# Fro116/RecommenderSystem

Measured on AMD Instinct MI355X. Metric: interactions/sec, higher is better.
Workload: dtype bf16

## Files before the change

recommendersystem_amd/csrc/elementwise.hip:

```cpp
#include "kernels.hpp"

namespace rsys {

thread_local DetScratch g_det;

__global__ void reduce_parts_kernel(const float* __restrict__ part, int nparts, long long stride, int n, float* dst) {
  const int c = blockIdx.x * blockDim.x + threadIdx.x;
  if (c >= n) return;
  float acc = 0.f;
  for (int b = 0; b < nparts; ++b) acc += part[(long long)b * stride + c];
  dst[c] += acc;
}
__global__ void reduce_parts_stage_kernel(const float* __restrict__ part, int nparts, long long stride, int n, float* out) {
  const int c = blockIdx.x * blockDim.x + threadIdx.x, chunk = blockIdx.y;
  if (c >= n) return;
  const int b0 = chunk * 32, b1 = min(nparts, b0 + 32);
  float acc = 0.f;
  for (int b = b0; b < b1; ++b) acc += part[(long long)b * stride + c];
  out[(long long)chunk * n + c] = acc;
}
int launch_reduce_parts(const float* part, int nparts, long long stride, int n, float* dst, hipStream_t s) {
  if (nparts <= 0 || n <= 0) return RSYS_OK;
  if (nparts > 64 && g_det.tmp != nullptr) {
    const int chunks = (nparts + 31) / 32;
// ... 429 lines not shown
template int launch_dropout<float>(const float*, float*, long long, float, unsigned long long, unsigned int, int, hipStream_t);

struct SelectBatch { const float* w[4]; int* idx[4]; float* stats[4]; int* npos[4]; };
__global__ __launch_bounds__(1024) void select_positions_kernel(SelectBatch sb, int N, int topk) {
  const float* __restrict__ w = sb.w[blockIdx.x];
  int* idx = sb.idx[blockIdx.x]; float* stats = sb.stats[blockIdx.x]; int* npos_out = sb.npos[blockIdx.x];
  __shared__ int wave_tot[16];
  __shared__ float red[16];
  const int t = threadIdx.x, l = t & 63, wv = t >> 6;
  const int per = (N + 1023) / 1024;
  const int i0 = t * per, i1 = min(N, i0 + per);
  int cnt = 0; float wall = 0.f;
  for (int i = i0; i < i1; ++i) { float x = w[i]; cnt += x > 0.f; wall += x; }
  int inc = cnt;
#pragma unroll
  for (int o = 1; o < 64; o <<= 1) { int v = __shfl_up(inc, o, 64); if (l >= o) inc += v; }
  if (l == 63) wave_tot[wv] = inc;
  __syncthreads();
  int base = 0, npos = 0;
  for (int k = 0; k < 16; ++k) { int v = wave_tot[k]; if (k < wv) base += v; npos += v; }
  int rank = base + inc - cnt;
  float wsel = 0.f;
  for (int i = i0; i < i1; ++i) {
    float x = w[i];
    int slot = x > 0.f ? rank : npos + (i - rank);
    if (slot < topk) { idx[slot] = i; wsel += x; }
    rank += x > 0.f;
  }
  wsel = block_sum(wsel, red);
  wall = block_sum(wall, red);
  if (t == 0) { stats[0] = wsel; stats[1] = wall; if (npos_out) *npos_out = min(npos, topk); }
}
constexpr int SEL_CHUNKS = 32;
__global__ __launch_bounds__(256) void select_count_kernel(SelectBatch sb, int N, int* __restrict__ counts, float* __restrict__ wsums) {
  __shared__ float red[16];
  const int task = blockIdx.x / SEL_CHUNKS, ch = blockIdx.x % SEL_CHUNKS;
  const float* __restrict__ w = sb.w[task];
  const int per = (N + SEL_CHUNKS - 1) / SEL_CHUNKS, i0 = ch * per, i1 = min(N, i0 + per);
  float cnt = 0.f, wall = 0.f;
  for (int i = i0 + threadIdx.x; i < i1; i += 256) { const float x = w[i]; cnt += x > 0.f ? 1.f : 0.f; wall += x; }
  cnt = block_sum(cnt, red);
  wall = block_sum(wall, red);
  if (threadIdx.x == 0) { counts[blockIdx.x] = (int)cnt; wsums[blockIdx.x] = wall; }
}
__global__ __launch_bounds__(256) void select_place_kernel(SelectBatch sb, int N, int topk, const int* __restrict__ counts, const float* __restrict__ wsums,
                                                           float* __restrict__ wsel_part) {
  __shared__ int wave_tot[4];
  __shared__ float red[16];
  const int task = blockIdx.x / SEL_CHUNKS, ch = blockIdx.x % SEL_CHUNKS;
  const float* __restrict__ w = sb.w[task];
  int* idx = sb.idx[task];
  const int t = threadIdx.x, l = t & 63, wv = t >> 6;
  int before = 0, npos = 0;
  for (int k = 0; k < SEL_CHUNKS; ++k) { const int v = counts[task * SEL_CHUNKS + k]; if (k < ch) before += v; npos += v; }
  const int per = (N + SEL_CHUNKS - 1) / SEL_CHUNKS, i0 = ch * per, i1 = min(N, i0 + per);
  float wsel = 0.f;
  int rank0 = before;
  for (int j0 = i0; j0 < i1; j0 += 256) {
    const int i = j0 + t;
    const float x = i < i1 ? w[i] : 0.f;
    const int pos = x > 0.f ? 1 : 0;
    int inc = pos;
#pragma unroll
    for (int o = 1; o < 64; o <<= 1) { const int v = __shfl_up(inc, o, 64); if (l >= o) inc += v; }
    __syncthreads();
    if (l == 63) wave_tot[wv] = inc;
    __syncthreads();
    int base = 0, tot = 0;
#pragma unroll
    for (int k = 0; k < 4; ++k) { const int v = wave_tot[k]; if (k < wv) base += v; tot += v; }
    const int rank = rank0 + base + inc - pos;
    if (i < i1) {
      const int slot = pos ? rank : npos + (i - rank);
      if (slot < topk) { idx[slot] = i; wsel += x; }
    }
    rank0 += tot;
  }
  wsel = block_sum(wsel, red);
  if (t == 0) wsel_part[blockIdx.x] = wsel;
}
__global__ void select_finish_kernel(SelectBatch sb, int ntask, int topk, const int* __restrict__ counts, const float* __restrict__ wsums,
                                     const float* __restrict__ wsel_part) {
  const int task = threadIdx.x;
  if (task >= ntask) return;
  int npos = 0; float wall = 0.f, wsel = 0.f;
  for (int k = 0; k < SEL_CHUNKS; ++k) { npos += counts[task * SEL_CHUNKS + k]; wall += wsums[task * SEL_CHUNKS + k]; wsel += wsel_part[task * SEL_CHUNKS + k]; }
  sb.stats[task][0] = wsel; sb.stats[task][1] = wall;
  if (sb.npos[task]) *sb.npos[task] = min(npos, topk);
}
int launch_select_positions_chunked(int ntask, const float* const* w, int N, int topk, int* const* idx, float* const* stats, int* const* npos_out,
                                    void* scratch, hipStream_t s) {
  ARG_CHECK(topk <= N && ntask >= 1 && ntask <= 4 && scratch != nullptr, "select_positions: topk > N or more than 4 tasks");
  SelectBatch sb{};
  for (int i = 0; i < ntask; ++i) { sb.w[i] = w[i]; sb.idx[i] = idx[i]; sb.stats[i] = stats[i]; sb.npos[i] = npos_out[i]; }
  int* counts = (int*)scratch; float* wsums = (float*)scratch + 4 * SEL_CHUNKS; float* wsel = (float*)scratch + 8 * SEL_CHUNKS;
  hipLaunchKernelGGL(select_count_kernel, dim3(ntask * SEL_CHUNKS), dim3(256), 0, s, sb, N, counts, wsums);
  hipLaunchKernelGGL(select_place_kernel, dim3(ntask * SEL_CHUNKS), dim3(256), 0, s, sb, N, topk, counts, wsums, wsel);
  hipLaunchKernelGGL(select_finish_kernel, dim3(1), dim3(64), 0, s, sb, ntask, topk, counts, wsums, wsel);
  HIP_CHECK(hipGetLastError());
  return RSYS_OK;
}

int launch_select_positions(const float* w, int N, int topk, int* idx, float* stats, int* npos_out, hipStream_t s) {
  const float* ws[1] = {w}; int* is[1] = {idx}; float* st[1] = {stats}; int* np[1] = {npos_out};
  return launch_select_positions_batch(1, ws, N, topk, is, st, np, s);
}
int launch_select_positions_batch(int ntask, const float* const* w, int N, int topk, int* const* idx, float* const* stats,
                                  int* const* npos_out, hipStream_t s) {
  ARG_CHECK(topk <= N && ntask >= 1 && ntask <= 4, "select_positions: topk > N or more than 4 tasks");
  SelectBatch sb{};
  for (int i = 0; i < ntask; ++i) { sb.w[i] = w[i]; sb.idx[i] = idx[i]; sb.stats[i] = stats[i]; sb.npos[i] = npos_out[i]; }
  hipLaunchKernelGGL(select_positions_kernel, dim3(ntask), dim3(1024), 0, s, sb, N, topk);
  HIP_CHECK(hipGetLastError());
  return RSYS_OK;
}

template <typename T>
__global__ void gather_rows_kernel(const T* __restrict__ src, long long ld, const int* __restrict__ idx, int parity, T* dst, int n, int D) {
  const int row = (blockIdx.x * blockDim.x + threadIdx.x) >> 6, l = threadIdx.x & 63;
  if (row >= n) return;
  constexpr int E = 16 / sizeof(T);
  const uint4* s4 = (const uint4*)(src + (2LL * idx[row] + parity) * ld);
  uint4* d4 = (uint4*)(dst + (long long)row * D);
  for (int c = l; c < D / E; c += 64) d4[c] = s4[c];
}
template <typename T>
int launch_gather_rows(const T* src, long long ld, const int* idx, int parity, T* dst, int n, int D, hipStream_t s) {
  ARG_CHECK((D * sizeof(T)) % 16 == 0 && (ld * sizeof(T)) % 16 == 0, "gather_rows: rows must be 16-byte multiples");
  hipLaunchKernelGGL((gather_rows_kernel<T>), dim3(div_up(n, 4)), dim3(256), 0, s, src, ld, idx, parity, dst, n, D);
  HIP_CHECK(hipGetLastError());
  return RSYS_OK;
}
template int launch_gather_rows<bf16>(const bf16*, long long, const int*, int, bf16*, int, int, hipStream_t);
template int launch_gather_rows<float>(const float*, long long, const int*, int, float*, int, int, hipStream_t);

__global__ void scatter_rows_add_kernel(const float* __restrict__ src, const int* __restrict__ idx, int parity, float* dst, long long ld, int n, int D,
                                        const int* __restrict__ npos) {
  const int row = (blockIdx.x * blockDim.x + threadIdx.x) >> 6, l = threadIdx.x & 63;
  if (row >= n || (npos != nullptr && row >= *npos)) return;
  const float4* s4 = (const float4*)(src + (long long)row * D);
  float4* d4 = (float4*)(dst + (2LL * idx[row] + parity) * ld);
  for (int c = l; c < (D >> 2); c += 64) {
    float4 a = d4[c], b = s4[c];
    a.x += b.x; a.y += b.y; a.z += b.z; a.w += b.w;
    d4[c] = a;
  }
}
int launch_scatter_rows_add(const float* src, const int* idx, int parity, float* dst, long long ld, int n, int D, hipStream_t s, const int* npos) {
  hipLaunchKernelGGL(scatter_rows_add_kernel, dim3(div_up(n, 4)), dim3(256), 0, s, src, idx, parity, dst, ld, n, D, npos);
  HIP_CHECK(hipGetLastError());
  return RSYS_OK;
}

template <typename T>
__global__ __launch_bounds__(256) void ce_kernel(T* logits, long long ldl, int V, const int* __restrict__ idx,
                                                 const float* __restrict__ label, const float* __restrict__ weight,
                                                 const int* __restrict__ position, const float* __restrict__ stats,
                                                 const int* __restrict__ npos, float task_w, float* loss_out, float* part) {
  __shared__ float red[16];
  constexpr int E = 16 / sizeof(T);
  const int row = blockIdx.x, t = threadIdx.x;
  if (npos != nullptr && row >= ((*npos + 127) & ~127)) return;
  T* lr = logits + (long long)row * ldl;
  const int i = idx[row];
  const float w = weight[i], lab = label[i];
  const int nchunks = (int)(ldl / E);
  const float lw = lab * w;
  if (lw == 0.f) {
    for (int c = t; c < nchunks; c += 256) ((uint4*)lr)[c] = make_uint4(0, 0, 0, 0);
    return;
  }
  float m = -3.0e38f, ssum = 0.f;
  for (int c = t; c < nchunks; c += 256) {
    uint4 raw = ((const uint4*)lr)[c];
    const T* e = (const T*)&raw;
#pragma unroll
    for (int k = 0; k < E; ++k) {
      if (c * E + k < V) {
        float x = to_f32(e[k]);
        if (x > m) { ssum = ssum * __expf(m - x) + 1.f; m = x; }
        else ssum += __expf(x - m);
      }
    }
  }
  const float gm = block_max(m, red);
  ssum = block_sum(ssum * __expf(m - gm), red);
  const float lse = gm + logf(ssum);
  const int tgt = position[i];
  const float xt = to_f32(lr[tgt]);
  __syncthreads();
  if (t == 0) {
    if (part != nullptr) part[row] = (lse - xt) * lw;
    else atomicAdd(loss_out, (lse - xt) * lw);
  }
  const float coef = task_w * lw / fmaxf(stats[0], 1e-8f);
  for (int c = t; c < nchunks; c += 256) {
    uint4 raw = ((const uint4*)lr)[c];
    T* e = (T*)&raw;
#pragma unroll
    for (int k = 0; k < E; ++k) {
      int col = c * E + k;
      float x = to_f32(e[k]);
      float gl = col < V ? coef * (__expf(x - lse) - (col == tgt ? 1.f : 0.f)) : 0.f;
      e[k] = from_f32<T>(gl);
    }
    ((uint4*)lr)[c] = raw;
  }
}
template <typename T>
int launch_ce_fwd_bwd(T* logits, long long ldl, int n, int V, const int* idx, const float* label, const float* weight,
                      const int* position, const float* stats, const int* npos, float task_w, float* loss_out, hipStream_t s) {
  ARG_CHECK((ldl * sizeof(T)) % 16 == 0 && ldl >= V, "ce: ldl");
  if (n <= 0) return RSYS_OK;
  float* part = det_part(n);
  if (part != nullptr) HIP_CHECK(hipMemsetAsync(part, 0, (size_t)n * 4, s));
  hipLaunchKernelGGL((ce_kernel<T>), dim3(n), dim3(256), 0, s, logits, ldl, V, idx, label, weight, position, stats, npos, task_w, loss_out, part);
  HIP_CHECK(hipGetLastError());
  if (part != nullptr) return launch_reduce_parts(part, n, 1, 1, loss_out, s);
  return RSYS_OK;
}
template int launch_ce_fwd_bwd<bf16>(bf16*, long long, int, int, const int*, const float*, const float*, const int*, const float*, const int*, float, float*, hipStream_t);
template int launch_ce_fwd_bwd<float>(float*, long long, int, int, const int*, const float*, const float*, const int*, const float*, const int*, float, float*, hipStream_t);

template <typename T>
__global__ __launch_bounds__(256) void rating_tail_kernel(T* z, const T* __restrict__ hact, int n, int D,
                                                          const float* __restrict__ w2, const float* __restrict__ b2,
                                                          const int* __restrict__ idx, const float* __restrict__ label,
                                                          const float* __restrict__ weight, const float* __restrict__ stats,
                                                          float rating_mean, float task_w, int evaluate, float* loss_out,
                                                          float* dw2, float* db2, float* db0, float* part, const int* __restrict__ npos) {
  extern __shared__ __attribute__((aligned(16))) float sds[];
  const int l = threadIdx.x & 63, w = threadIdx.x >> 6;
  const int nacc = part != nullptr ? 4 * 2 * D + 16 : 2 * D;
  for (int c = threadIdx.x; c < nacc; c += 256) sds[c] = 0.f;
  __syncthreads();
  float* const mine = part != nullptr ? sds + w * 2 * D : sds;
  float l0 = 0.f, l1 = 0.f, l2 = 0.f, gb2 = 0.f;
  const float inv_ws = 1.f / fmaxf(stats[0], 1e-8f);
  if (npos != nullptr) n = min(n, (*npos + 127) & ~127);
  for (int row = blockIdx.x * 4 + w; row < n; row += gridDim.x * 4) {
    const int i = idx[row];
    const float wt = weight[i], tgt = label[i] - rating_mean;
    const T* hr = hact + (long long)row * D;
    T* zr = z + (long long)row * D;
    float acc = 0.f;
    for (int c = l; c < D; c += 64) acc += to_f32(hr[c]) * w2[c];
    acc = wave_sum(acc);
    const float pred = acc + b2[0];
    const float e1 = pred - tgt;
    l0 += e1 * e1 * wt; l1 += tgt * tgt * wt; l2 += (-pred - tgt) * (-pred - tgt) * wt;
    const float dpred = evaluate ? 0.f : task_w * 2.f * e1 * wt * inv_ws;
    gb2 += dpred;
    for (int c = l; c < D; c += 64) {
      float zz = to_f32(zr[c]);
      float gp = 0.5f * (1.f + erff(zz * 0.70710678118654752f)) + zz * __expf(-0.5f * zz * zz) * 0.3989422804014327f;
      float dz = dpred * w2[c] * gp;
      zr[c] = from_f32<T>(dz);
      if (dpred != 0.f) {
        if (part != nullptr) { mine[c] += dpred * to_f32(hr[c]); mine[D + c] += dz; }
        else { atomicAdd(&sds[c], dpred * to_f32(hr[c])); atomicAdd(&sds[D + c], dz); }
      }
    }
  }
  if (part != nullptr) {
    float* sc = sds + 4 * 2 * D;
    if (l == 0) { sc[w * 4 + 0] = gb2; sc[w * 4 + 1] = l0; sc[w * 4 + 2] = l1; sc[w * 4 + 3] = l2; }
    __syncthreads();
    float* pr = part + (long long)blockIdx.x * (2 * D + 4);
    for (int c = threadIdx.x; c < 2 * D; c += 256) pr[c] = ((sds[c] + sds[2 * D + c]) + sds[4 * D + c]) + sds[6 * D + c];
    if (threadIdx.x < 4) pr[2 * D + threadIdx.x] = ((sc[threadIdx.x] + sc[4 + threadIdx.x]) + sc[8 + threadIdx.x]) + sc[12 + threadIdx.x];
    return;
  }
  __syncthreads();
  if (!evaluate) {
    for (int c = threadIdx.x; c < D; c += 256) {
      if (sds[c] != 0.f) atomicAdd(&dw2[c], sds[c]);
      if (sds[D + c] != 0.f) atomicAdd(&db0[c], sds[D + c]);
    }
    if (l == 0 && gb2 != 0.f) atomicAdd(db2, gb2);
  }
  if (l == 0) {
    if (l0 != 0.f) atomicAdd(&loss_out[0], l0);
    if (l1 != 0.f) atomicAdd(&loss_out[1], l1);
    if (l2 != 0.f) atomicAdd(&loss_out[2], l2);
  }
}
template <typename T>
int launch_rating_tail(T* z, const T* hact, int n, int D, const float* w2, const float* b2, const int* idx,
                       const float* label, const float* weight, const float* stats, float rating_mean, float task_w,
                       int evaluate, float* loss_out, float* dw2, float* db2, float* db0, hipStream_t s, const int* npos) {
  if (n <= 0) return RSYS_OK;
  int grid = std::min(div_up(n, 4), 512);
  const long long prow = 2LL * D + 4;
  float* part = det_part(grid * prow);
  hipLaunchKernelGGL((rating_tail_kernel<T>), dim3(grid), dim3(256), (part ? 8 * D + 16 : 2 * D) * sizeof(float), s, z, hact, n, D, w2, b2, idx,
                     label, weight, stats, rating_mean, task_w, evaluate, loss_out, dw2, db2, db0, part, npos);
  HIP_CHECK(hipGetLastError());
  if (part != nullptr) {
    int rc = RSYS_OK;
    if (!evaluate) {
      rc = launch_reduce_parts(part, grid, prow, D, dw2, s);
      if (rc == RSYS_OK) rc = launch_reduce_parts(part + D, grid, prow, D, db0, s);
      if (rc == RSYS_OK) rc = launch_reduce_parts(part + 2 * D, grid, prow, 1, db2, s);
    }
    return rc == RSYS_OK ? launch_reduce_parts(part + 2 * D + 1, grid, prow, 3, loss_out, s) : rc;
  }
  return RSYS_OK;
}
template int launch_rating_tail<bf16>(bf16*, const bf16*, int, int, const float*, const float*, const int*, const float*, const float*, const float*, float, float, int, float*, float*, float*, float*, hipStream_t, const int*);
template int launch_rating_tail<float>(float*, const float*, int, int, const float*, const float*, const int*, const float*, const float*, const float*, float, float, int, float*, float*, float*, float*, hipStream_t, const int*);

template <typename T>
__global__ void widen_kernel(const T* __restrict__ src, float* __restrict__ dst, long long n) {
  for (long long i = (long long)blockIdx.x * blockDim.x + threadIdx.x; i < n; i += (long long)gridDim.x * blockDim.x) dst[i] = to_f32(src[i]);
}
template <typename T>
int launch_widen(const T* src, float* dst, long long n, hipStream_t s) {
  const int blocks = (int)std::min<long long>((n + 255) / 256, 8192);
  hipLaunchKernelGGL((widen_kernel<T>), dim3(blocks), dim3(256), 0, s, src, dst, n);
  HIP_CHECK(hipGetLastError());
  return RSYS_OK;
}
template int launch_widen<bf16>(const bf16*, float*, long long, hipStream_t);
template int launch_widen<float>(const float*, float*, long long, hipStream_t);
template <typename T>
__global__ void rowdot_kernel(const T* __restrict__ h, const float* __restrict__ w, const float* __restrict__ b, float* out, int n, int D) {
  const int row = (blockIdx.x * blockDim.x + threadIdx.x) >> 6, l = threadIdx.x & 63;
  if (row >= n) return;
  const T* hr = h + (long long)row * D;
  float acc = 0.f;
  for (int c = l; c < D; c += 64) acc += to_f32(hr[c]) * w[c];
  acc = wave_sum(acc);
  if (l == 0) out[row] = acc + b[0];
}
template <typename T>
int launch_rowdot(const T* h, const float* w, const float* b, float* out, int n, int D, hipStream_t s) {
  hipLaunchKernelGGL((rowdot_kernel<T>), dim3(div_up(n, 4)), dim3(256), 0, s, h, w, b, out, n, D);
  HIP_CHECK(hipGetLastError());
  return RSYS_OK;
}
template int launch_rowdot<bf16>(const bf16*, const float*, const float*, float*, int, int, hipStream_t);
template int launch_rowdot<float>(const float*, const float*, const float*, float*, int, int, hipStream_t);

template <typename TS>
__global__ void colsum_kernel(const TS* __restrict__ src, long long ld, long long rows, int cols, float* dst, int rows_per_block, float* part) {
  const int c = blockIdx.x * blockDim.x + threadIdx.x;
  if (c >= cols) return;
  const long long r0 = (long long)blockIdx.y * rows_per_block, r1 = min(rows, r0 + rows_per_block);
  float acc = 0.f;
  for (long long r = r0; r < r1; ++r) acc += to_f32(src[r * ld + c]);
  if (part != nullptr) part[(long long)blockIdx.y * cols + c] = acc;
  else if (acc != 0.f) atomicAdd(&dst[c], acc);
}
template <typename TS>
static int colsum_any(const TS* src, long long ld, long long rows, int cols, float* dst, hipStream_t s) {
  int rpb = (int)std::max<long long>(64, (rows + 511) / 512);
  dim3 grid(div_up(cols, 256), div_up(rows, rpb));
  float* part = det_part((long long)grid.y * cols);
  hipLaunchKernelGGL((colsum_kernel<TS>), grid, dim3(256), 0, s, src, ld, rows, cols, dst, rpb, part);
  HIP_CHECK(hipGetLastError());
  if (part != nullptr) return launch_reduce_parts(part, (int)grid.y, cols, cols, dst, s);
  return RSYS_OK;
}
int launch_colsum_add(const float* src, long long ld, long long rows, int cols, float* dst, hipStream_t s) {
  return colsum_any<float>(src, ld, rows, cols, dst, s);
}

__global__ __launch_bounds__(1024) void cast_colsum_kernel(const float* __restrict__ src, bf16* __restrict__ dst, long long rows, int D,
                                                           float* colsum, int rows_per_block, float* part) {
  __shared__ float red[2048];
  const int cg = D >> 2;
  const int c = (threadIdx.x % cg) * 4, lane_r = threadIdx.x / cg, nr = 1024 / cg;
  const long long r0 = (long long)blockIdx.x * rows_per_block, r1 = min(rows, r0 + rows_per_block);
  float4 acc = make_float4(0, 0, 0, 0);
  long long r = r0 + lane_r;
  for (; r + 3 * nr < r1; r += 4 * nr) {
    float4 v[4];
#pragma unroll
    for (int u = 0; u < 4; ++u) v[u] = *(const float4*)(src + (r + u * nr) * D + c);
#pragma unroll
    for (int u = 0; u < 4; ++u) {
      bf16x4 o; o[0] = (bf16)v[u].x; o[1] = (bf16)v[u].y; o[2] = (bf16)v[u].z; o[3] = (bf16)v[u].w;
      *(bf16x4*)(dst + (r + u * nr) * D + c) = o;
      acc.x += v[u].x; acc.y += v[u].y; acc.z += v[u].z; acc.w += v[u].w;
    }
  }
  for (; r < r1; r += nr) {
    const float4 v = *(const float4*)(src + r * D + c);
    bf16x4 o; o[0] = (bf16)v.x; o[1] = (bf16)v.y; o[2] = (bf16)v.z; o[3] = (bf16)v.w;
    *(bf16x4*)(dst + r * D + c) = o;
    acc.x += v.x; acc.y += v.y; acc.z += v.z; acc.w += v.w;
  }
  if (lane_r < 2) *(float4*)&red[lane_r * D + c] = acc;
  __syncthreads();
  for (int base = 2; base < nr; base += 2) {
    if (lane_r >= base && lane_r < base + 2) {
      float4 o = *(float4*)&red[(lane_r - base) * D + c];
      o.x += acc.x; o.y += acc.y; o.z += acc.z; o.w += acc.w;
      *(float4*)&red[(lane_r - base) * D + c] = o;
    }
    __syncthreads();
  }
  for (int cc = threadIdx.x; cc < D; cc += 1024) {
    const float v = red[cc] + (nr > 1 ? red[D + cc] : 0.f);
    if (part != nullptr) part[(long long)blockIdx.x * D + cc] = v;
    else if (v != 0.f) atomicAdd(&colsum[cc], v);
  }
}
int launch_cast_colsum(const float* src, bf16* dst, long long rows, int D, float* colsum, hipStream_t s) {
  ARG_CHECK(D % 4 == 0 && D <= 1024 && 1024 % (D >> 2) == 0, "cast_colsum: D/4 must divide 1024, D <= 1024");
  const int rpb = (int)std::max<long long>(32, (rows + 511) / 512);
  const int grid = div_up(rows, rpb);
  float* part = det_part((long long)grid * D);
  hipLaunchKernelGGL(cast_colsum_kernel, dim3(grid), dim3(1024), 0, s, src, dst, rows, D, colsum, rpb, part);
  HIP_CHECK(hipGetLastError());
  if (part != nullptr) return launch_reduce_parts(part, grid, D, D, colsum, s);
  return RSYS_OK;
}

__global__ __launch_bounds__(256) void cast_transpose_colsum_kernel(const float* __restrict__ src, bf16* __restrict__ dstT, long long rows, int D,
                                                                    long long ldt, float* colsum, int rows_per_block, float* part) {
  __shared__ unsigned short tile[64][72];
  __shared__ float red[16][64];
  const int t = threadIdx.x;
  const int lr = t >> 4, c4 = (t & 15) * 4;
  const int oc = t >> 2, or8 = (t & 3) * 16;
  const long long r0 = (long long)blockIdx.x * rows_per_block;
  const long long rend = min((rows + 63) & ~63LL, r0 + rows_per_block);
  for (int ct = 0; ct < D / 64; ++ct) {
    float4 acc = make_float4(0, 0, 0, 0);
    for (long long rb = r0; rb < rend; rb += 64) {
      float4 v[4];
#pragma unroll
      for (int i = 0; i < 4; ++i) {
        const long long r = rb + 4 * lr + i;
        v[i] = r < rows ? *(const float4*)(src + r * D + ct * 64 + c4) : make_float4(0, 0, 0, 0);
        acc.x += v[i].x; acc.y += v[i].y; acc.z += v[i].z; acc.w += v[i].w;
      }
      {
        bf16x4 o;
        o[0] = (bf16)v[0].x; o[1] = (bf16)v[1].x; o[2] = (bf16)v[2].x; o[3] = (bf16)v[3].x; *(bf16x4*)&tile[c4 + 0][4 * lr] = o;
        o[0] = (bf16)v[0].y; o[1] = (bf16)v[1].y; o[2] = (bf16)v[2].y; o[3] = (bf16)v[3].y; *(bf16x4*)&tile[c4 + 1][4 * lr] = o;
        o[0] = (bf16)v[0].z; o[1] = (bf16)v[1].z; o[2] = (bf16)v[2].z; o[3] = (bf16)v[3].z; *(bf16x4*)&tile[c4 + 2][4 * lr] = o;
        o[0] = (bf16)v[0].w; o[1] = (bf16)v[1].w; o[2] = (bf16)v[2].w; o[3] = (bf16)v[3].w; *(bf16x4*)&tile[c4 + 3][4 * lr] = o;
      }
      __syncthreads();
      {
        const uint4 q0 = *(const uint4*)&tile[oc][or8], q1 = *(const uint4*)&tile[oc][or8 + 8];
        uint4* d = (uint4*)(dstT + (long long)(ct * 64 + oc) * ldt + rb + or8);
        d[0] = q0; d[1] = q1;
      }
      __syncthreads();
    }
    *(float4*)&red[lr][c4] = acc;
    __syncthreads();
    if (t < 64) {
      float v = 0.f;
#pragma unroll
      for (int k = 0; k < 16; ++k) v += red[k][t];
      if (part != nullptr) part[(long long)blockIdx.x * D + ct * 64 + t] = v;
      else if (v != 0.f) atomicAdd(&colsum[ct * 64 + t], v);
    }
    __syncthreads();
  }
}
int launch_cast_transpose_colsum(const float* src, bf16* dstT, long long rows, int D, long long ldt, float* colsum, hipStream_t s) {
  ARG_CHECK(D % 64 == 0 && ldt % 8 == 0 && ldt >= ((rows + 63) & ~63LL), "cast_transpose_colsum: D % 64, ldt % 8, ldt >= rows rounded up to 64");
  const long long chunks = (rows + 63) / 64;
  const int cpb = (int)std::max<long long>(1, (chunks + 2047) / 2048);
  const int grid = (int)((chunks + cpb - 1) / cpb);
  float* part = det_part((long long)grid * D);
  hipLaunchKernelGGL(cast_transpose_colsum_kernel, dim3(grid), dim3(256), 0, s, src, dstT, rows, D, ldt, colsum, cpb * 64, part);
  HIP_CHECK(hipGetLastError());
  if (part != nullptr) return launch_reduce_parts(part, grid, D, D, colsum, s);
  return RSYS_OK;
}

__global__ void embedding_scatter_kernel(const float* __restrict__ gx0, BatchDev b, int V, int D, float* gE) {
  const int n = (blockIdx.x * blockDim.x + threadIdx.x) >> 6, l = threadIdx.x & 63;
  if (n >= b.N) return;
  int id = b.m_matchedid[n];
  id = id == -1 ? V : id;
  const float* src = gx0 + (long long)(2 * n) * D;
  float* dst = gE + (long long)id * D;
  for (int c = l; c < D; c += 64) atomicAdd(&dst[c], src[c]);
}
int launch_embedding_scatter_add(const float* gx0, const BatchDev& b, int V, int D, float* gE, hipStream_t s) {
  hipLaunchKernelGGL(embedding_scatter_kernel, dim3(div_up(b.N, 4)), dim3(256), 0, s, gx0, b, V, D, gE);
  HIP_CHECK(hipGetLastError());
  return RSYS_OK;
}

__global__ __launch_bounds__(256) void action_small_bwd_kernel(const float* __restrict__ gf, BatchDev b, SmallParams sp,
                                                               float* g_cos, float* g_sin, float* g_status, float* g_gender,
                                                               float* g_source) {
  __shared__ float acc[4 + 16 * 4 + 16 * 4 + 16 * 16];
  const int NG = (sp.n_gender + 1) * 4, NS = (sp.n_source + 1) * 4, NST = (sp.n_status + 1) * 16;
  float* a_g = acc + 4; float* a_s = a_g + 64; float* a_st = a_s + 64;
  for (int c = threadIdx.x; c < 4 + 64 + 64 + 256; c += 256) acc[c] = 0.f;
  __syncthreads();
  for (int i = blockIdx.x * blockDim.x + threadIdx.x; i < b.N; i += gridDim.x * blockDim.x) {
    const float* g = gf + (long long)i * 32;
    float p0, p1; double ts;
    periodic_args(b.time[i], sp.min_ts, p0, p1, ts);
    atomicAdd(&acc[0], -sinf(p0 + sp.per_cos[0]) * g[1]);
    atomicAdd(&acc[1], -sinf(p1 + sp.per_cos[1]) * g[2]);
    atomicAdd(&acc[2], cosf(p0 + sp.per_sin[0]) * g[3]);
    atomicAdd(&acc[3], cosf(p1 + sp.per_sin[1]) * g[4]);
    int gi = b.gender[i]; gi = gi == -1 ? sp.n_gender : gi;
    int si = b.source[i]; si = si == -1 ? sp.n_source : si;
    int st = b.m_status[i]; st = st == -1 ? sp.n_status : st;
#pragma unroll
    for (int k = 0; k < 4; ++k) atomicAdd(&a_g[gi * 4 + k], g[5 + k]);
#pragma unroll
    for (int k = 0; k < 4; ++k) atomicAdd(&a_s[si * 4 + k], g[9 + k]);
#pragma unroll
    for (int k = 0; k < 16; ++k) atomicAdd(&a_st[st * 16 + k], g[15 + k]);
  }
// ... 58 lines not shown
```

Baseline: 1.631 million.

## Register-resident CE kernel, vectorized rating tail, and float4 column-sum kernel

The cross-entropy kernel now keeps the whole logit row in registers across larger blocks. It computes max and sum-exp in separate passes rather than with an online rescale, and writes gradients without re-reading global memory. The rating tail kernel vectorizes its loads and keeps w2 and the per-lane accumulators in registers, replacing shared-memory atomics with a per-wave serialized reduction on a smaller grid. A new float4 colsum kernel uses a shared-memory row reduction for the nondeterministic path; the deterministic paths keep the older kernels, and the changes add register pressure and more template variants.

```diff
diff --git a/recommendersystem_amd/csrc/elementwise.hip b/recommendersystem_amd/csrc/elementwise.hip
--- a/recommendersystem_amd/csrc/elementwise.hip
+++ b/recommendersystem_amd/csrc/elementwise.hip
@@ -605,36 +605,92 @@
   return RSYS_OK;
 }
 
-template <typename T>
-__global__ __launch_bounds__(256) void ce_kernel(T* logits, long long ldl, int V, const int* __restrict__ idx,
-                                                 const float* __restrict__ label, const float* __restrict__ weight,
-                                                 const int* __restrict__ position, const float* __restrict__ stats,
-                                                 const int* __restrict__ npos, float task_w, float* loss_out, float* part) {
+constexpr float CE_NEG = -3.0e38f;
+
+__device__ __forceinline__ bool ce_row_skipped(int row, const int* __restrict__ npos) {
+  return npos != nullptr && row >= ((*npos + 127) & ~127);
+}
+__device__ __forceinline__ void ce_clear_row(void* lr, int nchunks) {
+  for (int c = threadIdx.x; c < nchunks; c += blockDim.x) ((uint4*)lr)[c] = make_uint4(0, 0, 0, 0);
+}
+__device__ __forceinline__ unsigned& ce_word(uint4& q, int j) { return j == 0 ? q.x : j == 1 ? q.y : j == 2 ? q.z : q.w; }
+template <typename T>
+__device__ __forceinline__ float ce_get(uint4& q, int k) {
+  if constexpr (is_bf16<T>::value) return __uint_as_float(k & 1 ? ce_word(q, k >> 1) & 0xffff0000u : ce_word(q, k >> 1) << 16);
+  else return __uint_as_float(ce_word(q, k));
+}
+template <typename T>
+__device__ __forceinline__ void ce_set_neg(uint4& q, int k) {
+  if constexpr (is_bf16<T>::value) ce_word(q, k >> 1) = k & 1 ? (ce_word(q, k >> 1) & 0xffffu) | 0xff620000u : (ce_word(q, k >> 1) & 0xffff0000u) | 0xff62u;
+  else ce_word(q, k) = __float_as_uint(CE_NEG);
+}
+template <typename T>
+__device__ __forceinline__ void ce_grad_chunk(uint4& raw, int cbase, int V, int tgt, float lse, float coef) {
+  constexpr int E = 16 / sizeof(T);
+  float g[E];
+  if ((unsigned)(tgt - cbase) >= (unsigned)E && cbase + E <= V) {
+#pragma unroll
+    for (int k = 0; k < E; ++k) g[k] = coef * (__expf(ce_get<T>(raw, k) - lse) - 0.f);
+  } else {
+#pragma unroll
+    for (int k = 0; k < E; ++k) {
+      const int col = cbase + k;
+      const float gl = coef * (__expf(ce_get<T>(raw, k) - lse) - (col == tgt ? 1.f : 0.f));
+      g[k] = col < V ? gl : 0.f;
+    }
+  }
+#pragma unroll
+  for (int j = 0; j < 4; ++j) {
+    if constexpr (is_bf16<T>::value) { bf16x2 pk; pk[0] = (bf16)g[2 * j]; pk[1] = (bf16)g[2 * j + 1]; ce_word(raw, j) = __builtin_bit_cast(unsigned, pk); }
+    else ce_word(raw, j) = __float_as_uint(g[j]);
+  }
+}
+
+__device__ __forceinline__ void ce_tie(float& a, uint4& q) {
+  asm volatile("" : "+v"(a), "+v"(q.x), "+v"(q.y), "+v"(q.z), "+v"(q.w));
+}
+
+template <typename T, int NT, int NC>
+__global__ __launch_bounds__(NT) void ce_kernel(T* logits, long long ldl, int V, const int* __restrict__ idx,
+                                                const float* __restrict__ label, const float* __restrict__ weight,
+                                                const int* __restrict__ position, const float* __restrict__ stats,
+                                                const int* __restrict__ npos, float task_w, float* loss_out, float* part) {
   __shared__ float red[16];
   constexpr int E = 16 / sizeof(T);
   const int row = blockIdx.x, t = threadIdx.x;
-  if (npos != nullptr && row >= ((*npos + 127) & ~127)) return;
+  if (ce_row_skipped(row, npos)) return;
   T* lr = logits + (long long)row * ldl;
   const int i = idx[row];
-  const float w = weight[i], lab = label[i];
-  const int nchunks = (int)(ldl / E);
-  const float lw = lab * w;
-  if (lw == 0.f) {
-    for (int c = t; c < nchunks; c += 256) ((uint4*)lr)[c] = make_uint4(0, 0, 0, 0);
-    return;
-  }
-  float m = -3.0e38f, ssum = 0.f;
-  for (int c = t; c < nchunks; c += 256) {
-    uint4 raw = ((const uint4*)lr)[c];
-    const T* e = (const T*)&raw;
-#pragma unroll
-    for (int k = 0; k < E; ++k) {
-      if (c * E + k < V) {
-        float x = to_f32(e[k]);
-        if (x > m) { ssum = ssum * __expf(m - x) + 1.f; m = x; }
-        else ssum += __expf(x - m);
-      }
-    }
+  const int nchunks = (int)(ldl / E), vchunks = (V + E - 1) / E;
+  const float lw = label[i] * weight[i];
+  if (lw == 0.f) { ce_clear_row(lr, nchunks); return; }
+  uint4 r[NC];
+#pragma unroll
+  for (int u = 0; u < NC; ++u) {
+    r[u] = ((const uint4*)lr)[min(t + u * NT, vchunks - 1)];
+  }
+  float m = CE_NEG;
+#pragma unroll
+  for (int u = 0; u < NC; ++u) {
+    const int cbase = (t + u * NT) * E;
+    ce_tie(m, r[u]);
+    if (cbase + E > V) {
+#pragma unroll
+      for (int k = 0; k < E; ++k) if (cbase + k >= V) ce_set_neg<T>(r[u], k);
+    }
+    float m0 = ce_get<T>(r[u], 0), m1 = ce_get<T>(r[u], 1);
+#pragma unroll
+    for (int k = 2; k < E; k += 2) { m0 = fmaxf(m0, ce_get<T>(r[u], k)); m1 = fmaxf(m1, ce_get<T>(r[u], k + 1)); }
+    m = fmaxf(m, fmaxf(m0, m1));
+  }
+  float ssum = 0.f;
+#pragma unroll
+  for (int u = 0; u < NC; ++u) {
+    ce_tie(ssum, r[u]);
+    float s0 = __expf(ce_get<T>(r[u], 0) - m), s1 = __expf(ce_get<T>(r[u], 1) - m);
+#pragma unroll
+    for (int k = 2; k < E; k += 2) { s0 += __expf(ce_get<T>(r[u], k) - m); s1 += __expf(ce_get<T>(r[u], k + 1) - m); }
+    ssum += s0 + s1;
   }
   const float gm = block_max(m, red);
   ssum = block_sum(ssum * __expf(m - gm), red);
@@ -646,20 +702,78 @@
     if (part != nullptr) part[row] = (lse - xt) * lw;
     else atomicAdd(loss_out, (lse - xt) * lw);
   }
+  float coef = task_w * lw / fmaxf(stats[0], 1e-8f);
+#pragma unroll
+  for (int u = 0; u < NC; ++u) {
+    const int c = t + u * NT;
+    ce_tie(coef, r[u]);
+    if (c < vchunks) {
+      ce_grad_chunk<T>(r[u], c * E, V, tgt, lse, coef);
+      ((uint4*)lr)[c] = r[u];
+    }
+  }
+  for (int c = vchunks + t; c < nchunks; c += NT) ((uint4*)lr)[c] = make_uint4(0, 0, 0, 0);
+}
+
+constexpr int CE2_NT = 256, CE2_U = 4;
+template <typename T>
+__global__ __launch_bounds__(CE2_NT) void ce_two_pass_kernel(T* logits, long long ldl, int V, const int* __restrict__ idx,
+                                                             const float* __restrict__ label, const float* __restrict__ weight,
+                                                             const int* __restrict__ position, const float* __restrict__ stats,
+                                                             const int* __restrict__ npos, float task_w, float* loss_out, float* part) {
+  __shared__ float red[16];
+  constexpr int E = 16 / sizeof(T);
+  const int row = blockIdx.x, t = threadIdx.x;
+  if (ce_row_skipped(row, npos)) return;
+  T* lr = logits + (long long)row * ldl;
+  const int i = idx[row];
+  const int nchunks = (int)(ldl / E);
+  const float lw = label[i] * weight[i];
+  if (lw == 0.f) { ce_clear_row(lr, nchunks); return; }
+  float m = -3.0e38f, ssum = 0.f;
+  for (int c0 = t; c0 < nchunks; c0 += CE2_U * CE2_NT) {
+    uint4 raw[CE2_U];
+#pragma unroll
+    for (int u = 0; u < CE2_U; ++u) raw[u] = ((const uint4*)lr)[min(c0 + u * CE2_NT, nchunks - 1)];
+#pragma unroll
+    for (int u = 0; u < CE2_U; ++u) {
+      const int c = c0 + u * CE2_NT;
+#pragma unroll
+      for (int k = 0; k < E; ++k) {
+        if (c < nchunks && c * E + k < V) {
+          float x = ce_get<T>(raw[u], k);
+          if (x > m) { ssum = ssum * __expf(m - x) + 1.f; m = x; }
+          else ssum += __expf(x - m);
+        }
+      }
+    }
+  }
+  const float gm = block_max(m, red);
+  ssum = block_sum(ssum * __expf(m - gm), red);
+  const float lse = gm + logf(ssum);
+  const int tgt = position[i];
+  const float xt = to_f32(lr[tgt]);
+  __syncthreads();
+  if (t == 0) {
+    if (part != nullptr) part[row] = (lse - xt) * lw;
+    else atomicAdd(loss_out, (lse - xt) * lw);
+  }
   const float coef = task_w * lw / fmaxf(stats[0], 1e-8f);
-  for (int c = t; c < nchunks; c += 256) {
-    uint4 raw = ((const uint4*)lr)[c];
-    T* e = (T*)&raw;
-#pragma unroll
-    for (int k = 0; k < E; ++k) {
-      int col = c * E + k;
-      float x = to_f32(e[k]);
-      float gl = col < V ? coef * (__expf(x - lse) - (col == tgt ? 1.f : 0.f)) : 0.f;
-      e[k] = from_f32<T>(gl);
-    }
-    ((uint4*)lr)[c] = raw;
-  }
-}
+  for (int c0 = t; c0 < nchunks; c0 += CE2_U * CE2_NT) {
+    uint4 raw[CE2_U];
+#pragma unroll
+    for (int u = 0; u < CE2_U; ++u) raw[u] = ((const uint4*)lr)[min(c0 + u * CE2_NT, nchunks - 1)];
+#pragma unroll
+    for (int u = 0; u < CE2_U; ++u) {
+      const int c = c0 + u * CE2_NT;
+      if (c < nchunks) {
+        ce_grad_chunk<T>(raw[u], c * E, V, tgt, lse, coef);
+        ((uint4*)lr)[c] = raw[u];
+      }
+    }
+  }
+}
+constexpr int CE_REG_CHUNKS = 16 * 1024;
 template <typename T>
 int launch_ce_fwd_bwd(T* logits, long long ldl, int n, int V, const int* idx, const float* label, const float* weight,
                       const int* position, const float* stats, const int* npos, float task_w, float* loss_out, hipStream_t s) {
@@ -667,7 +781,15 @@
   if (n <= 0) return RSYS_OK;
   float* part = det_part(n);
   if (part != nullptr) HIP_CHECK(hipMemsetAsync(part, 0, (size_t)n * 4, s));
-  hipLaunchKernelGGL((ce_kernel<T>), dim3(n), dim3(256), 0, s, logits, ldl, V, idx, label, weight, position, stats, npos, task_w, loss_out, part);
+  const long long vchunks = ((long long)V * sizeof(T) + 15) / 16;
+#define CE_LAUNCH(kernel, nt) hipLaunchKernelGGL((kernel), dim3(n), dim3(nt), 0, s, logits, ldl, V, idx, label, weight, position, stats, npos, task_w, loss_out, part)
+  if (part != nullptr) CE_LAUNCH((ce_two_pass_kernel<T>), CE2_NT);
+  else if (vchunks <= 4 * 256) CE_LAUNCH((ce_kernel<T, 256, 4>), 256);
+  else if (vchunks <= 8 * 1024) CE_LAUNCH((ce_kernel<T, 1024, 8>), 1024);
+  else if (vchunks <= 12 * 1024) CE_LAUNCH((ce_kernel<T, 1024, 12>), 1024);
+  else if (vchunks <= CE_REG_CHUNKS) CE_LAUNCH((ce_kernel<T, 1024, 16>), 1024);
+  else CE_LAUNCH((ce_two_pass_kernel<T>), CE2_NT);
+#undef CE_LAUNCH
   HIP_CHECK(hipGetLastError());
   if (part != nullptr) return launch_reduce_parts(part, n, 1, 1, loss_out, s);
   return RSYS_OK;
@@ -675,19 +797,136 @@
 template int launch_ce_fwd_bwd<bf16>(bf16*, long long, int, int, const int*, const float*, const float*, const int*, const float*, const int*, float, float*, hipStream_t);
 template int launch_ce_fwd_bwd<float>(float*, long long, int, int, const int*, const float*, const float*, const int*, const float*, const int*, float, float*, hipStream_t);
 
-template <typename T>
+constexpr int RATING_TAIL_GRID = 128;
+template <typename T>
+__device__ __forceinline__ void load8(const T* p, float (&v)[8]);
+template <>
+__device__ __forceinline__ void load8<bf16>(const bf16* p, float (&v)[8]) {
+  const bf16x8 r = *(const bf16x8*)p;
+#pragma unroll
+  for (int k = 0; k < 8; ++k) v[k] = (float)r[k];
+}
+template <>
+__device__ __forceinline__ void load8<float>(const float* p, float (&v)[8]) {
+  const float4 a = *(const float4*)p, b = *(const float4*)(p + 4);
+  v[0] = a.x; v[1] = a.y; v[2] = a.z; v[3] = a.w; v[4] = b.x; v[5] = b.y; v[6] = b.z; v[7] = b.w;
+}
+__device__ __forceinline__ void store8(bf16* p, const float (&v)[8]) {
+  bf16x8 r;
+#pragma unroll
+  for (int k = 0; k < 8; ++k) r[k] = (bf16)v[k];
+  *(bf16x8*)p = r;
+}
+__device__ __forceinline__ void store8(float* p, const float (&v)[8]) {
+  *(float4*)p = make_float4(v[0], v[1], v[2], v[3]);
+  *(float4*)(p + 4) = make_float4(v[4], v[5], v[6], v[7]);
+}
+template <typename T, int NJ>
 __global__ __launch_bounds__(256) void rating_tail_kernel(T* z, const T* __restrict__ hact, int n, int D,
                                                           const float* __restrict__ w2, const float* __restrict__ b2,
                                                           const int* __restrict__ idx, const float* __restrict__ label,
                                                           const float* __restrict__ weight, const float* __restrict__ stats,
                                                           float rating_mean, float task_w, int evaluate, float* loss_out,
-                                                          float* dw2, float* db2, float* db0, float* part, const int* __restrict__ npos) {
+                                                          float* dw2, float* db2, float* db0, const int* __restrict__ npos) {
+  extern __shared__ __attribute__((aligned(16))) float sds[];
+  const int l = threadIdx.x & 63, w = threadIdx.x >> 6, ngroups = D >> 3;
+  float w2r[NJ][8], aw[NJ][8], ab[NJ][8];
+#pragma unroll
+  for (int j = 0; j < NJ; ++j) {
+    const int g = l + 64 * j;
+#pragma unroll
+    for (int k = 0; k < 8; ++k) { w2r[j][k] = 0.f; aw[j][k] = 0.f; ab[j][k] = 0.f; }
+    if (g < ngroups) load8<float>(w2 + g * 8, w2r[j]);
+  }
+  float l0 = 0.f, l1 = 0.f, l2 = 0.f, gb2 = 0.f;
+  const float inv_ws = 1.f / fmaxf(stats[0], 1e-8f);
+  if (npos != nullptr) n = min(n, (*npos + 127) & ~127);
+  for (int row = blockIdx.x * 4 + w; row < n; row += gridDim.x * 4) {
+    const int i = idx[row];
+    const float wt = weight[i], tgt = label[i] - rating_mean;
+    const T* hr = hact + (long long)row * D;
+    T* zr = z + (long long)row * D;
+    float h[NJ][8], zz[NJ][8];
+#pragma unroll
+    for (int j = 0; j < NJ; ++j) {
+      const int g = l + 64 * j;
+#pragma unroll
+      for (int k = 0; k < 8; ++k) { h[j][k] = 0.f; zz[j][k] = 0.f; }
+      if (g < ngroups) { load8<T>(hr + g * 8, h[j]); load8<T>(zr + g * 8, zz[j]); }
+    }
+    float acc = 0.f;
+#pragma unroll
+    for (int j = 0; j < NJ; ++j)
+#pragma unroll
+      for (int k = 0; k < 8; ++k) acc += h[j][k] * w2r[j][k];
+    acc = wave_sum(acc);
+    const float pred = acc + b2[0];
+    const float e1 = pred - tgt;
+    l0 += e1 * e1 * wt; l1 += tgt * tgt * wt; l2 += (-pred - tgt) * (-pred - tgt) * wt;
+    const float dpred = evaluate ? 0.f : task_w * 2.f * e1 * wt * inv_ws;
+    gb2 += dpred;
+#pragma unroll
+    for (int j = 0; j < NJ; ++j) {
+      const int g = l + 64 * j;
+      if (g < ngroups) {
+        float dz[8];
+#pragma unroll
+        for (int k = 0; k < 8; ++k) {
+          const float v = zz[j][k];
+          const float gp = 0.5f * (1.f + erff(v * 0.70710678118654752f)) + v * __expf(-0.5f * v * v) * 0.3989422804014327f;
+          dz[k] = dpred * w2r[j][k] * gp;
+        }
+        store8(zr + g * 8, dz);
+        if (dpred != 0.f) {
+#pragma unroll
+          for (int k = 0; k < 8; ++k) { aw[j][k] += dpred * h[j][k]; ab[j][k] += dz[k]; }
+        }
+      }
+    }
+  }
+  float* sc = sds + 2 * D;
+  for (int ww = 0; ww < 4; ++ww) {
+    if (w == ww) {
+#pragma unroll
+      for (int j = 0; j < NJ; ++j) {
+        const int g = l + 64 * j;
+        if (g < ngroups) {
+#pragma unroll
+          for (int k = 0; k < 8; ++k) {
+            const int c = g * 8 + k;
+            sds[c] = ww == 0 ? aw[j][k] : sds[c] + aw[j][k];
+            sds[D + c] = ww == 0 ? ab[j][k] : sds[D + c] + ab[j][k];
+          }
+        }
+      }
+      if (l == 0) {
+        sc[0] = ww == 0 ? gb2 : sc[0] + gb2; sc[1] = ww == 0 ? l0 : sc[1] + l0;
+        sc[2] = ww == 0 ? l1 : sc[2] + l1;   sc[3] = ww == 0 ? l2 : sc[3] + l2;
+      }
+    }
+    __syncthreads();
+  }
+  if (!evaluate) {
+    for (int c = threadIdx.x; c < D; c += 256) {
+      if (sds[c] != 0.f) atomicAdd(&dw2[c], sds[c]);
+      if (sds[D + c] != 0.f) atomicAdd(&db0[c], sds[D + c]);
+    }
+    if (threadIdx.x == 0 && sc[0] != 0.f) atomicAdd(db2, sc[0]);
+  }
+  if (threadIdx.x >= 1 && threadIdx.x < 4 && sc[threadIdx.x] != 0.f) atomicAdd(&loss_out[threadIdx.x - 1], sc[threadIdx.x]);
+}
+template <typename T>
+__global__ __launch_bounds__(256) void rating_tail_ordered_kernel(T* z, const T* __restrict__ hact, int n, int D,
+                                                                  const float* __restrict__ w2, const float* __restrict__ b2,
+                                                                  const int* __restrict__ idx, const float* __restrict__ label,
+                                                                  const float* __restrict__ weight, const float* __restrict__ stats,
+                                                                  float rating_mean, float task_w, int evaluate, float* part,
+                                                                  const int* __restrict__ npos) {
   extern __shared__ __attribute__((aligned(16))) float sds[];
   const int l = threadIdx.x & 63, w = threadIdx.x >> 6;
-  const int nacc = part != nullptr ? 4 * 2 * D + 16 : 2 * D;
-  for (int c = threadIdx.x; c < nacc; c += 256) sds[c] = 0.f;
+  for (int c = threadIdx.x; c < 4 * 2 * D + 16; c += 256) sds[c] = 0.f;
   __syncthreads();
-  float* const mine = part != nullptr ? sds + w * 2 * D : sds;
+  float* const mine = sds + w * 2 * D;
   float l0 = 0.f, l1 = 0.f, l2 = 0.f, gb2 = 0.f;
   const float inv_ws = 1.f / fmaxf(stats[0], 1e-8f);
   if (npos != nullptr) n = min(n, (*npos + 127) & ~127);
@@ -709,45 +948,35 @@
       float gp = 0.5f * (1.f + erff(zz * 0.70710678118654752f)) + zz * __expf(-0.5f * zz * zz) * 0.3989422804014327f;
       float dz = dpred * w2[c] * gp;
       zr[c] = from_f32<T>(dz);
-      if (dpred != 0.f) {
-        if (part != nullptr) { mine[c] += dpred * to_f32(hr[c]); mine[D + c] += dz; }
-        else { atomicAdd(&sds[c], dpred * to_f32(hr[c])); atomicAdd(&sds[D + c], dz); }
-      }
-    }
-  }
-  if (part != nullptr) {
-    float* sc = sds + 4 * 2 * D;
-    if (l == 0) { sc[w * 4 + 0] = gb2; sc[w * 4 + 1] = l0; sc[w * 4 + 2] = l1; sc[w * 4 + 3] = l2; }
-    __syncthreads();
-    float* pr = part + (long long)blockIdx.x * (2 * D + 4);
-    for (int c = threadIdx.x; c < 2 * D; c += 256) pr[c] = ((sds[c] + sds[2 * D + c]) + sds[4 * D + c]) + sds[6 * D + c];
-    if (threadIdx.x < 4) pr[2 * D + threadIdx.x] = ((sc[threadIdx.x] + sc[4 + threadIdx.x]) + sc[8 + threadIdx.x]) + sc[12 + threadIdx.x];
-    return;
-  }
+      if (dpred != 0.f) { mine[c] += dpred * to_f32(hr[c]); mine[D + c] += dz; }
+    }
+  }
+  float* sc = sds + 4 * 2 * D;
+  if (l == 0) { sc[w * 4 + 0] = gb2; sc[w * 4 + 1] = l0; sc[w * 4 + 2] = l1; sc[w * 4 + 3] = l2; }
   __syncthreads();
-  if (!evaluate) {
-    for (int c = threadIdx.x; c < D; c += 256) {
-      if (sds[c] != 0.f) atomicAdd(&dw2[c], sds[c]);
-      if (sds[D + c] != 0.f) atomicAdd(&db0[c], sds[D + c]);
-    }
-    if (l == 0 && gb2 != 0.f) atomicAdd(db2, gb2);
-  }
-  if (l == 0) {
-    if (l0 != 0.f) atomicAdd(&loss_out[0], l0);
-    if (l1 != 0.f) atomicAdd(&loss_out[1], l1);
-    if (l2 != 0.f) atomicAdd(&loss_out[2], l2);
-  }
+  float* pr = part + (long long)blockIdx.x * (2 * D + 4);
+  for (int c = threadIdx.x; c < 2 * D; c += 256) pr[c] = ((sds[c] + sds[2 * D + c]) + sds[4 * D + c]) + sds[6 * D + c];
+  if (threadIdx.x < 4) pr[2 * D + threadIdx.x] = ((sc[threadIdx.x] + sc[4 + threadIdx.x]) + sc[8 + threadIdx.x]) + sc[12 + threadIdx.x];
 }
 template <typename T>
 int launch_rating_tail(T* z, const T* hact, int n, int D, const float* w2, const float* b2, const int* idx,
                        const float* label, const float* weight, const float* stats, float rating_mean, float task_w,
                        int evaluate, float* loss_out, float* dw2, float* db2, float* db0, hipStream_t s, const int* npos) {
   if (n <= 0) return RSYS_OK;
-  int grid = std::min(div_up(n, 4), 512);
+  const bool ordered = g_det.part != nullptr;
+  const int grid = std::min(div_up(n, 4), ordered ? 512 : RATING_TAIL_GRID);
   const long long prow = 2LL * D + 4;
   float* part = det_part(grid * prow);
-  hipLaunchKernelGGL((rating_tail_kernel<T>), dim3(grid), dim3(256), (part ? 8 * D + 16 : 2 * D) * sizeof(float), s, z, hact, n, D, w2, b2, idx,
-                     label, weight, stats, rating_mean, task_w, evaluate, loss_out, dw2, db2, db0, part, npos);
+  if (part != nullptr) {
+    hipLaunchKernelGGL((rating_tail_ordered_kernel<T>), dim3(grid), dim3(256), (8 * D + 16) * sizeof(float), s, z, hact, n, D, w2, b2, idx,
+                       label, weight, stats, rating_mean, task_w, evaluate, part, npos);
+  } else {
+    ARG_CHECK(D >= 8 && D % 8 == 0 && D <= 2048, "rating_tail: D must be a multiple of 8 and <= 2048");
+    const int nj = div_up(D, 512);
+    auto* kernel = nj == 1 ? rating_tail_kernel<T, 1> : nj == 2 ? rating_tail_kernel<T, 2> : rating_tail_kernel<T, 4>;
+    hipLaunchKernelGGL(kernel, dim3(grid), dim3(256), (size_t)prow * sizeof(float), s, z, hact, n, D, w2, b2, idx,
+                       label, weight, stats, rating_mean, task_w, evaluate, loss_out, dw2, db2, db0, npos);
+  }
   HIP_CHECK(hipGetLastError());
   if (part != nullptr) {
     int rc = RSYS_OK;
@@ -805,6 +1034,43 @@
   if (part != nullptr) part[(long long)blockIdx.y * cols + c] = acc;
   else if (acc != 0.f) atomicAdd(&dst[c], acc);
 }
+__global__ __launch_bounds__(1024) void colsum4_kernel(const float* __restrict__ src, long long ld, long long rows, int cols, float* dst,
+                                                       int rows_per_block, int cg) {
+  __shared__ float4 red[1024];
+  const int tx = threadIdx.x & (cg - 1), lane_r = threadIdx.x / cg, nr = 1024 / cg;
+  const int c = (blockIdx.x * cg + tx) * 4;
+  const long long r0 = (long long)blockIdx.y * rows_per_block, r1 = min(rows, r0 + rows_per_block);
+  float4 acc = make_float4(0, 0, 0, 0);
+  if (c < cols) {
+    long long r = r0 + lane_r;
+    for (; r + 7 * nr < r1; r += 8 * nr) {
+      float4 v[8];
+#pragma unroll
+      for (int u = 0; u < 8; ++u) v[u] = *(const float4*)(src + (r + u * nr) * ld + c);
+#pragma unroll
+      for (int u = 0; u < 8; ++u) { acc.x += v[u].x; acc.y += v[u].y; acc.z += v[u].z; acc.w += v[u].w; }
+    }
+    for (; r < r1; r += nr) {
+      const float4 v = *(const float4*)(src + r * ld + c);
+      acc.x += v.x; acc.y += v.y; acc.z += v.z; acc.w += v.w;
+    }
+  }
+  red[threadIdx.x] = acc;
+  __syncthreads();
+  if (lane_r == 0) {
+    for (int q = 1; q < nr; ++q) {
+      const float4 o = red[q * cg + tx];
+      acc.x += o.x; acc.y += o.y; acc.z += o.z; acc.w += o.w;
+    }
+    red[tx] = acc;
+  }
+  __syncthreads();
+  const int cc = blockIdx.x * cg * 4 + threadIdx.x;
+  if (threadIdx.x < cg * 4 && cc < cols) {
+    const float v = ((const float*)red)[threadIdx.x];
+    if (v != 0.f) atomicAdd(&dst[cc], v);
+  }
+}
 template <typename TS>
 static int colsum_any(const TS* src, long long ld, long long rows, int cols, float* dst, hipStream_t s) {
   int rpb = (int)std::max<long long>(64, (rows + 511) / 512);
@@ -816,7 +1082,14 @@
   return RSYS_OK;
 }
 int launch_colsum_add(const float* src, long long ld, long long rows, int cols, float* dst, hipStream_t s) {
-  return colsum_any<float>(src, ld, rows, cols, dst, s);
+  if (g_det.part != nullptr || ((uintptr_t)src & 15) != 0 || (ld & 3) != 0 || (cols & 3) != 0) return colsum_any<float>(src, ld, rows, cols, dst, s);
+  const int rpb = (int)std::max<long long>(128, (rows + 255) / 256);
+  int cg = 1;
+  while (cg < 256 && cg * 4 < cols) cg *= 2;
+  dim3 grid(div_up(cols, cg * 4), div_up(rows, rpb));
+  hipLaunchKernelGGL(colsum4_kernel, grid, dim3(1024), 0, s, src, ld, rows, cols, dst, rpb, cg);
+  HIP_CHECK(hipGetLastError());
+  return RSYS_OK;
 }
 
 __global__ __launch_bounds__(1024) void cast_colsum_kernel(const float* __restrict__ src, bf16* __restrict__ dst, long long rows, int D,
```

Result: no change. 1.645 million (median of 6 runs) (+0.8%).
